# fboehm/DBSLMM

Measured on AMD Instinct MI355X. Metric: SNPs solved/sec (whole node) + max-|Δβ| vs CPU ref, 1M SNP × 10k indiv, higher is better.
Workload: dtype f64

## Files before the change

dbslmm_amd/csrc/pcg.hip:

```cpp
#include <hip/hip_runtime.h>
#include <stdint.h>

namespace pcg {
constexpr int kT = 128;
constexpr int kRunMax = 8;
constexpr int kMaxNC = 4;
constexpr int kWaves = 4;
constexpr int kVS = kT + 8;
constexpr int kNDot = 5;
constexpr int kQS = 8;
constexpr int kThreads = 256;
constexpr int kFTb = 8;
constexpr int kFRows = kFTb * kT;
constexpr int kFPer = kFRows / kThreads;
constexpr int wave_lds_doubles(int nc) { return 3 * nc * kVS + 4 * nc * 64; }
constexpr size_t lds_bytes(int nc) { return sizeof(double) * kWaves * wave_lds_doubles(nc); }
}

struct PcgBlk {
    int32_t blk, row0, m, ms;
    int32_t ld, Tb, Ns, sco;
    int64_t matoff, vo, po, dof;
    int64_t off16;
    int32_t nc;
    int32_t mshift;
    int32_t fused;
    int32_t pad_;
};

struct PcgArgs {
    const PcgBlk* blk;
    const uint16_t* G16;
    const double* M;
    const int32_t* flags;
    const double* S;
    const double* rsd;
    const double* z;
    const int32_t* slot_out;
    const int32_t* blk_id;
    const double* dshift;
    double *X, *R, *P, *Sv, *W;
    double* U;
    double* part;
    double* dot;
    double* qs;
    int32_t* cnv;
    int32_t* itb;
    int32_t* done;
    int32_t* active;
    int32_t* fin;
    double* beta_s;
    double* beta_l;
    int32_t* status;
    double* mir_s;
    double* mir_l;
    int32_t* mir_st;
    int32_t* mir_flag;
    int32_t run_no;
    int64_t vstride;
    int64_t ns, nl, nbk;
    double tau, rn, c0, tol, inv_sqrt_n;
    int32_t ncopy;
    int32_t run;
    int32_t seed;
};

namespace pcg {

__device__ __forceinline__ void wave_fence() {
    __builtin_amdgcn_fence(__ATOMIC_RELEASE, "wavefront");
    __builtin_amdgcn_wave_barrier();
    __builtin_amdgcn_fence(__ATOMIC_ACQUIRE, "wavefront");
}

template <int Ctrl>
__device__ __forceinline__ double dpp_mov(double v) {
    const uint64_t b = __builtin_bit_cast(uint64_t, v);
    const int lo = __builtin_amdgcn_mov_dpp(static_cast<int>(b & 0xffffffffu), Ctrl, 0xf, 0xf, false);
    const int hi = __builtin_amdgcn_mov_dpp(static_cast<int>(b >> 32), Ctrl, 0xf, 0xf, false);
    return __builtin_bit_cast(double, (static_cast<uint64_t>(static_cast<uint32_t>(hi)) << 32) | static_cast<uint32_t>(lo));
}
template <int X>
__device__ __forceinline__ uint32_t swap_xor(uint32_t x, bool up) {
    if constexpr (X == 16) {
        const auto r = __builtin_amdgcn_permlane16_swap(x, x, false, false);
        return up ? r[0] : r[1];
    } else {
        const auto r = __builtin_amdgcn_permlane32_swap(x, x, false, false);
        return up ? r[0] : r[1];
    }
}
template <int X>
__device__ __forceinline__ double lane_xor(double v) {
#ifndef PCG_NO_DPP
    if constexpr (X == 1) return dpp_mov<0xB1>(v);
    else if constexpr (X == 2) return dpp_mov<0x4E>(v);
    else if constexpr (X == 4) return dpp_mov<0x1B>(dpp_mov<0x141>(v));
    else if constexpr (X == 8) return dpp_mov<0x128>(v);
#ifndef PCG_NO_PERMLANE
    else if constexpr (X == 16 || X == 32) {
        const uint64_t b = __builtin_bit_cast(uint64_t, v);
        const bool up = (__lane_id() & X) != 0;
        const uint32_t lo = swap_xor<X>(static_cast<uint32_t>(b & 0xffffffffu), up);
        const uint32_t hi = swap_xor<X>(static_cast<uint32_t>(b >> 32), up);
        return __builtin_bit_cast(double, (static_cast<uint64_t>(hi) << 32) | lo);
    }
#endif
    else
#endif
        return __shfl_xor(v, X);
}

template <int X2, int X1, int X0>
__device__ __forceinline__ double rscatter8(const double (&v)[8], int lane) {
    const bool h2 = (lane & X2) != 0, h1 = (lane & X1) != 0, h0 = (lane & X0) != 0;
    double u[4], w[2];
#pragma unroll
    for (int q = 0; q < 4; ++q) {
        const double send = h2 ? v[q] : v[q + 4], keep = h2 ? v[q + 4] : v[q];
        u[q] = keep + lane_xor<X2>(send);
    }
#pragma unroll
    for (int q = 0; q < 2; ++q) {
        const double send = h1 ? u[q] : u[q + 2], keep = h1 ? u[q + 2] : u[q];
        w[q] = keep + lane_xor<X1>(send);
    }
    const double send = h0 ? w[0] : w[1], keep = h0 ? w[1] : w[0];
    return keep + lane_xor<X0>(send);
}

__device__ __forceinline__ double wave_sum(double v) {
    v += lane_xor<32>(v);
    v += lane_xor<16>(v);
    v += lane_xor<8>(v);
    v += lane_xor<4>(v);
    v += lane_xor<2>(v);
    v += lane_xor<1>(v);
    return v;
}



__device__ __forceinline__ double ordered_sum(const double* __restrict__ p, int64_t st, int s0, int s1, double acc) {
    for (int s = s0; s < s1; s += 8) {
        double t[8];
#pragma unroll
        for (int u = 0; u < 8; ++u) t[u] = s + u < s1 ? p[static_cast<int64_t>(s + u) * st] : 0.0;
#pragma unroll
        for (int u = 0; u < 8; ++u) acc += t[u];
    }
    return acc;
}

__device__ __forceinline__ bool on_u16(const PcgArgs& a, const PcgBlk& B) {
    return a.G16 != nullptr && (a.flags[B.blk] & 1) == 0;
}

__device__ __forceinline__ double jdiag(const PcgArgs& a, const PcgBlk& B, int i, double dc) {
    return B.mshift ? 1.0 : i < B.ms ? a.c0 + dc : a.c0;
}
__device__ __forceinline__ double col_shift(const PcgArgs& a, const PcgBlk& B, int k) {
    return a.dshift[B.mshift ? a.seed : k];
}

__device__ __forceinline__ void put_beta(const PcgArgs& a, const PcgBlk& B, int i, int k, double x, bool mono) {
    const int so = a.slot_out[B.row0 + i];
    const double bv = mono ? __builtin_nan("") : x * a.inv_sqrt_n;
    if (so >= 0) {
        a.beta_s[k * a.ns + so] = bv;
        if (a.mir_s) a.mir_s[k * a.ns + so] = bv;
    } else {
        a.beta_l[k * a.nl - 1 - so] = bv;
        if (a.mir_l) a.mir_l[k * a.nl - 1 - so] = bv;
    }
}
__device__ __forceinline__ void put_status(const PcgArgs& a, const PcgBlk& B, int k, bool mono) {
    const int st = mono ? DBSLMM_BLOCK_MONOMORPHIC
                        : a.cnv[B.sco + k] == 0 ? DBSLMM_BLOCK_NOT_CONVERGED : DBSLMM_BLOCK_OK;
    const int64_t o = k * a.nbk + a.blk_id[B.blk];
    a.status[o] = st;
    if (a.mir_st) a.mir_st[o] = st;
}

__device__ __forceinline__ double cvt_lo(uint32_t w) {
    double g;
    uint32_t t;
    asm volatile("v_and_b32 %1, 0xffff, %2\n\tv_cvt_f64_u32 %0, %1" : "=v"(g), "=&v"(t) : "v"(w));
    return g;
}
__device__ __forceinline__ double cvt_hi(uint32_t w) {
    double g;
    uint32_t t;
    asm volatile("v_lshrrev_b32 %1, 16, %2\n\tv_cvt_f64_u32 %0, %1" : "=v"(g), "=&v"(t) : "v"(w));
    return g;
}

typedef uint32_t pcg_u4 __attribute__((ext_vector_type(4)));

__device__ __forceinline__ __amdgpu_buffer_rsrc_t g16_rsrc(const uint16_t* base, uint32_t bytes) {
    const uint64_t gb = reinterpret_cast<uint64_t>(base);
    const uint32_t lo = static_cast<uint32_t>(__builtin_amdgcn_readfirstlane(static_cast<int>(gb & 0xffffffffu)));
    const uint32_t hi = static_cast<uint32_t>(__builtin_amdgcn_readfirstlane(static_cast<int>(gb >> 32)));
    const int nb = __builtin_amdgcn_readfirstlane(static_cast<int>(bytes));
    return __builtin_amdgcn_make_buffer_rsrc(reinterpret_cast<void*>((static_cast<uint64_t>(hi) << 32) | lo),
                                             static_cast<short>(0), nb, 0x00020000);
}
constexpr uint32_t kG16Oob = 0x80000000u;

__device__ __forceinline__ void quad_mul16(const pcg_u4 (&raw)[8], bool diagq, int lane, int nc,
                                           const double* vI, const double* vJ, double* rsum, double* csum) {
    const int rg = lane >> 3, cg = lane & 7;
#pragma unroll 1
    for (int k = 0; k < nc; ++k) {
        double vi[8], vj[8], racc[8], cacc[8];
#pragma unroll
        for (int q = 0; q < 8; ++q) {
            vi[q] = vI[k * kVS + 8 * rg + q];
            vj[q] = vJ[k * kVS + 8 * cg + q];
            racc[q] = cacc[q] = 0.0;
        }
        if (!diagq) {
#pragma unroll
            for (int r = 0; r < 8; ++r)
#pragma unroll
                for (int c = 0; c < 8; ++c) {
                    const uint32_t w = raw[r][c >> 1];
                    const double g = (c & 1) ? cvt_hi(w) : cvt_lo(w);
                    racc[r] = __builtin_fma(g, vj[c], racc[r]);
                    cacc[c] = __builtin_fma(g, vi[r], cacc[c]);
                }
        } else {
#pragma unroll
            for (int r = 0; r < 8; ++r)
#pragma unroll
                for (int c = 0; c < 8; ++c) {
                    const uint32_t w = raw[r][c >> 1];
                    const double g = (c & 1) ? cvt_hi(w) : cvt_lo(w);
                    const int dd = 8 * (cg - rg) + c - r;
                    racc[r] = __builtin_fma(dd <= 0 ? g : 0.0, vj[c], racc[r]);
                    cacc[c] = __builtin_fma(dd < 0 ? g : 0.0, vi[r], cacc[c]);
                }
        }
        rsum[k * 64 + lane] += rscatter8<4, 2, 1>(racc, lane);
        csum[k * 64 + lane] += rscatter8<32, 16, 8>(cacc, lane);
    }
}

__device__ __forceinline__ void quad_mul64(const double* __restrict__ base, int64_t ld, int rows_ok, int cols_ok,
                                           bool diagq, int lane, int nc, const double* vI, const double* vJ,
                                           double* rsum, double* csum) {
    const int rg = lane >> 3, cg = lane & 7;
#pragma unroll 1
    for (int k = 0; k < nc; ++k) {
        double vi[8], vj[8], racc[8], cacc[8];
#pragma unroll
        for (int q = 0; q < 8; ++q) {
            vi[q] = vI[k * kVS + 8 * rg + q];
            vj[q] = vJ[k * kVS + 8 * cg + q];
            racc[q] = cacc[q] = 0.0;
        }
#pragma unroll 1
        for (int r = 0; r < 8; ++r)
#pragma unroll
            for (int c = 0; c < 8; ++c) {
                const double g = (r < rows_ok && c < cols_ok) ? base[r * ld + c] : 0.0;
                const int dd = 8 * (cg - rg) + c - r;
                const double gr = !diagq || dd <= 0 ? g : 0.0, gc = !diagq || dd < 0 ? g : 0.0;
#pragma unroll
                for (int q = 0; q < 8; ++q)
                    if (q == r) racc[q] = __builtin_fma(gr, vj[c], racc[q]);
                cacc[c] = __builtin_fma(gc, vi[r], cacc[c]);
            }
        rsum[k * 64 + lane] += rscatter8<4, 2, 1>(racc, lane);
        csum[k * 64 + lane] += rscatter8<32, 16, 8>(cacc, lane);
    }
}

__device__ __forceinline__ void stage_v(const PcgArgs& a, const PcgBlk& B, int T, int nc, int lane, double* v) {
    for (int k = 0; k < nc; ++k) {
        const double* src = a.U + k * a.vstride + B.vo + static_cast<int64_t>(T) * kT;
        const double x0 = src[lane], x1 = src[lane + 64];
        v[k * kVS + lane] = x0;
        v[k * kVS + lane + 64] = x1;
    }
}

__device__ __forceinline__ bool quad_active(const PcgBlk& B, int I, int J, int q) {
    const int qi = q >> 1, qj = q & 1;
    return !(J == I && qj > qi) && I * kT + 64 * qi < B.m && J * kT + 64 * qj < B.m;
}
__device__ __forceinline__ bool next_quad(const PcgBlk& B, int I, int J1, int& J, int& q) {
    for (;;) {
        if (++q == 4) {
            q = 0;
            if (++J > J1) return false;
        }
        if (quad_active(B, I, J, q)) return true;
    }
}

template <bool U16>
__device__ void symv_item(const PcgArgs& a, int4 item, int lane, double* vI, double* vJb, double* rsum,
                          double* csum) {
    const PcgBlk B = a.blk[item.x];
    if (a.done[item.x] || on_u16(a, B) != U16) return;
    const int I = item.y, J0 = item.z, J1 = item.w, nc = B.nc;
    const int64_t ld16 = static_cast<int64_t>(B.Tb) * kT;
    const int rg = lane >> 3, cg = lane & 7;
    auto vj_of = [&](int J) -> double* { return J == I ? vI : vJb + ((J - J0) & 1) * nc * kVS; };
    const __amdgpu_buffer_rsrc_t g16 =
        g16_rsrc(a.G16 + B.off16 + static_cast<int64_t>(I) * kT * ld16, U16 ? static_cast<uint32_t>(kT * ld16 * 2) : 0u);
    auto load = [&](int J, int q, pcg_u4 (&raw)[8], bool none) {
        if constexpr (U16) {
            const int i0 = 64 * (q >> 1) + 8 * rg, j0 = J * kT + 64 * (q & 1) + 8 * cg;
            const bool skip = none || j0 >= B.m || (J == I && (q == 0 || q == 3) && cg > rg);
            const uint32_t o = static_cast<uint32_t>((static_cast<int64_t>(i0) * ld16 + j0) * 2);
#pragma unroll
            for (int r = 0; r < 8; ++r)
                raw[r] = __builtin_amdgcn_raw_buffer_load_b128(
                    g16, (skip || I * kT + i0 + r >= B.m) ? kG16Oob : o + static_cast<uint32_t>(r * ld16 * 2), 0, 0);
        }
    };
    auto mult = [&](int J, int q, const pcg_u4 (&raw)[8]) {
        const int qi = q >> 1, qj = q & 1;
        const bool dq = J == I && qi == qj;
        const double* vj = vj_of(J);
        double* rs = rsum + qi * nc * 64;
        double* cs = csum + qj * nc * 64;
        if constexpr (U16) {
            quad_mul16(raw, dq, lane, nc, vI + 64 * qi, vj + 64 * qj, rs, cs);
        } else {
            const int ib = I * kT + 64 * qi + 8 * rg, jb = J * kT + 64 * qj + 8 * cg;
            quad_mul64(a.M + B.matoff + static_cast<int64_t>(ib) * B.ld + jb, B.ld, B.m - ib, B.m - jb, dq,
                       lane, nc, vI + 64 * qi, vj + 64 * qj, rs, cs);
        }
    };
    auto flush = [&](int J) {
        double* dst = a.part + B.po + (static_cast<int64_t>(J) * B.Ns + I) * nc * kT;
        for (int qj = 0; qj < 2; ++qj)
            for (int k = 0; k < nc; ++k) {
                dst[k * kT + 64 * qj + 8 * cg + rg] = csum[(qj * nc + k) * 64 + lane];
                csum[(qj * nc + k) * 64 + lane] = 0.0;
            }
    };
    pcg_u4 ra[8], rb[8];
    int J = J0, q = 0;
    load(J, q, ra, false);
    stage_v(a, B, I, nc, lane, vI);
    if (J != I) stage_v(a, B, J, nc, lane, vj_of(J));
    for (int t = 0; t < 2 * nc; ++t) rsum[t * 64 + lane] = csum[t * 64 + lane] = 0.0;
    wave_fence();
    auto step = [&](pcg_u4 (&cur)[8], pcg_u4 (&nxt)[8]) -> bool {
        int Jn = J, qn = q;
        const bool more = next_quad(B, I, J1, Jn, qn);
        load(more ? Jn : J, more ? qn : q, nxt, !more);
        if (more && Jn != J && Jn != I) stage_v(a, B, Jn, nc, lane, vj_of(Jn));
        mult(J, q, cur);
        if (!more || Jn != J) flush(J);
        wave_fence();
        J = Jn;
        q = qn;
        return more;
    };
    while (step(ra, rb) && step(rb, ra)) {
    }
    double* dst = a.part + B.po + (static_cast<int64_t>(I) * B.Ns + B.Tb + J0 / a.run) * nc * kT;
    for (int qi = 0; qi < 2; ++qi)
        for (int k = 0; k < nc; ++k) dst[k * kT + 64 * qi + 8 * rg + cg] = rsum[(qi * nc + k) * 64 + lane];
}

}

extern "C" __global__ __launch_bounds__(pcg::kThreads) void dbslmm_pcg_init(PcgArgs a, const int2* __restrict__ rows) {
    using namespace pcg;
    __shared__ double red[kThreads / 64][kMaxNC];
    __shared__ int mono_s;
    const int2 it = rows[blockIdx.x];
    const int bi = it.x, I = it.y, tid = threadIdx.x;
    const PcgBlk B = a.blk[bi];
    const bool u16 = on_u16(a, B);
    const int n = a.ncopy, nc = B.nc;
    if (I == 0) {
        if (tid == 0) mono_s = 0;
        __syncthreads();
        bool mono = false;
        for (int i = tid; i < B.m; i += kThreads) mono |= !(a.rsd[B.row0 + i] < INFINITY);
        if (mono) atomicOr(&mono_s, 1);
        __syncthreads();
        if (tid < n) {
            a.cnv[B.sco + tid] = 0;
            double* q = a.qs + static_cast<int64_t>(B.sco + tid) * kQS;
            q[4] = q[5] = 1.0;
        }
        if (tid == 0) {
            a.itb[bi] = 0;
            a.fin[bi] = 0;
            const bool fz = B.fused && u16;
            a.done[bi] = mono_s ? 2 : fz ? 3 : 0;
            if (!mono_s && !fz) atomicAdd(a.active, 1);
        }
    }
    const int r = tid & (kT - 1), h = tid >> 7, i = I * kT + r;
    const bool in = i < B.m;
    double sv[kMaxNC];
#pragma unroll
    for (int k = 0; k < kMaxNC; ++k) sv[k] = 0.0;
    for (int c = h; c < n; c += 2) {
        const int64_t o = c * a.vstride + B.vo + i;
        const double rhs = in ? a.z[B.row0 + i] : 0.0;
        a.X[o] = 0.0;
        a.P[o] = 0.0;
        if (c < nc) {
            a.Sv[o] = 0.0;
            a.W[o] = 0.0;
            a.R[o] = rhs;
            double uv = 0.0;
            if (in) {
                uv = rhs / jdiag(a, B, i, col_shift(a, B, c));
                if (u16) uv *= a.rsd[B.row0 + i];
            }
            a.U[o] = uv;
        }
    }
#pragma unroll
    for (int k = 0; k < kMaxNC; ++k)
        if (k < nc && (k & 1) == h && in && u16) {
            const double rhs = a.z[B.row0 + i];
            sv[k] = a.S[B.row0 + i] * a.rsd[B.row0 + i] * (rhs / jdiag(a, B, i, col_shift(a, B, k)));
        }
#pragma unroll
    for (int k = 0; k < kMaxNC; ++k) sv[k] = wave_sum(sv[k]);
    if ((tid & 63) == 0)
#pragma unroll
        for (int k = 0; k < kMaxNC; ++k) red[tid >> 6][k] = sv[k];
    __syncthreads();
    if (tid < nc) {
        const int hk = tid & 1;
        a.dot[B.dof + (static_cast<int64_t>(I) * kNDot + 4) * n + tid] = red[2 * hk][tid] + red[2 * hk + 1][tid];
    }
}

template <bool U16>
__device__ __forceinline__ void symv_body(const PcgArgs& a, const int4* __restrict__ items, int32_t n_items) {
    using namespace pcg;
    extern __shared__ double vlds[];
    const int wave = threadIdx.x >> 6, lane = threadIdx.x & 63;
    const int e = blockIdx.x * kWaves + wave;
    if (e >= n_items) return;
    const int nc = a.ncopy;
    double* w = vlds + wave * wave_lds_doubles(nc);
    symv_item<U16>(a, items[e], lane, w, w + nc * kVS, w + 3 * nc * kVS, w + 3 * nc * kVS + 2 * nc * 64);
}
#ifndef PCG_SYMV_WAVES
#define PCG_SYMV_WAVES 2
#endif
extern "C" __global__ __launch_bounds__(pcg::kThreads) __attribute__((amdgpu_waves_per_eu(PCG_SYMV_WAVES, 8)))
void dbslmm_pcg_symv16(PcgArgs a, const int4* __restrict__ items, int32_t n_items) {
    symv_body<true>(a, items, n_items);
}
extern "C" __global__ __launch_bounds__(pcg::kThreads)
void dbslmm_pcg_symv64(PcgArgs a, const int4* __restrict__ items, int32_t n_items) {
    symv_body<false>(a, items, n_items);
}

extern "C" __global__ __launch_bounds__(pcg::kThreads) void dbslmm_pcg_rows(PcgArgs a, const int2* __restrict__ rows) {
    using namespace pcg;
    __shared__ double red[kThreads / 64][kMaxNC][4];
    __shared__ double sig[kMaxNC];
    const int2 it = rows[blockIdx.x];
    const int bi = it.x, I = it.y, tid = threadIdx.x;
    if (a.done[bi]) return;
    const PcgBlk B = a.blk[bi];
    const bool u16 = on_u16(a, B);
    const int n = a.ncopy, nc = B.nc;
    if (tid < nc)
        sig[tid] = ordered_sum(a.dot + B.dof + 4 * n + tid, kNDot * n, 0, B.Tb, 0.0);
    __syncthreads();
    const int r = tid & (kT - 1), h = tid >> 7, i = I * kT + r;
    const bool in = i < B.m;
    const double Si = in ? a.S[B.row0 + i] : 0.0, ri = in ? a.rsd[B.row0 + i] : 0.0;
    const int nrun = (I + a.run) / a.run;
    double dv[kMaxNC][4];
#pragma unroll
    for (int k = 0; k < kMaxNC; ++k)
#pragma unroll
        for (int f = 0; f < 4; ++f) dv[k][f] = 0.0;
#pragma unroll
    for (int k = 0; k < kMaxNC; ++k) {
        if (k >= n || (k & 1) != h) continue;
        const int64_t o = k * a.vstride + B.vo + i;
        if (k < nc) {
            const double* pp = a.part + B.po + static_cast<int64_t>(I) * B.Ns * nc * kT + k * kT + r;
            double y = ordered_sum(pp, nc * kT, I, B.Tb, 0.0);
            y = ordered_sum(pp, nc * kT, B.Tb, B.Tb + nrun, y);
            const double dc = col_shift(a, B, k);
            const double rv = a.R[o];
            const double u = in ? rv / jdiag(a, B, i, dc) : 0.0;
            const double sh = i < B.ms ? dc : 0.0;
            double w = 0.0;
            if (in) {
                if (u16) w = a.tau * a.rn * ri * __builtin_fma(-Si, sig[k] * a.rn, y) + (1.0 - a.tau + sh) * u;
                else w = y + sh * u;
            }
            a.W[o] = w;
            dv[k][0] = rv * u;
            dv[k][1] = w * u;
            dv[k][2] = rv * rv;
        }
        const double xv = a.X[o];
        dv[k][3] = xv * xv;
    }
#pragma unroll
    for (int k = 0; k < kMaxNC; ++k)
#pragma unroll
        for (int f = 0; f < 4; ++f) dv[k][f] = wave_sum(dv[k][f]);
    if ((tid & 63) == 0)
#pragma unroll
        for (int k = 0; k < kMaxNC; ++k)
#pragma unroll
            for (int f = 0; f < 4; ++f) red[tid >> 6][k][f] = dv[k][f];
    __syncthreads();
    if (tid < 4 * n) {
        const int k = tid >> 2, f = tid & 3, hk = k & 1;
        if (f == 3 || k < nc)
            a.dot[B.dof + (static_cast<int64_t>(I) * kNDot + f) * n + k] = red[2 * hk][k][f] + red[2 * hk + 1][k][f];
    }
    if (I == 0 && tid == 0) a.itb[bi] += 1;
}

extern "C" __global__ __launch_bounds__(pcg::kThreads) void dbslmm_pcg_update(PcgArgs a, const int2* __restrict__ rows) {
    using namespace pcg;
    __shared__ double tot[kMaxNC][4];
    __shared__ double coef[kMaxNC][3];
    __shared__ double seedc[2];
    __shared__ int run_s[kMaxNC];
    __shared__ double red[kThreads / 64][kMaxNC];
    const int2 it = rows[blockIdx.x];
    const int bi = it.x, I = it.y, tid = threadIdx.x;
    if (a.done[bi]) return;
    const PcgBlk B = a.blk[bi];
    const bool u16 = on_u16(a, B);
    const int n = a.ncopy, nc = B.nc;
    const int itn = a.itb[bi] - 1;
    const int par = itn & 1;
    if (tid < 4 * n) {
        const int k = tid >> 2, f = tid & 3;
        tot[k][f] = (f == 3 || k < nc) ? ordered_sum(a.dot + B.dof + f * n + k, kNDot * n, 0, B.Tb, 0.0) : 0.0;
    }
    __syncthreads();
    if (B.mshift) {
        if (tid == 0) {
            const double gam = tot[0][0], del = tot[0][1];
            const double* q = a.qs + static_cast<int64_t>(B.sco) * kQS;
            double al, be = 0.0;
            if (itn == 0) {
                al = gam / del;
            } else {
                be = gam / q[2 * par];
                al = gam / (del - be * gam / q[2 * par + 1]);
            }
            seedc[0] = al;
            seedc[1] = be;
        }
        __syncthreads();
        if (tid < n) {
            const int c = tid;
            double* q = a.qs + static_cast<int64_t>(B.sco + c) * kQS;
            const double al = seedc[0], be = seedc[1];
            const double zk = q[4 + 2 * par], zk1 = q[4 + 2 * par + 1];
            const double rr = tot[0][2] * zk * zk, xx = tot[c][3];
            const double t = a.tol * (a.dshift[c] + 1.0 - a.tau);
            const bool conv = a.cnv[B.sco + c] != 0 || rr == 0.0 || rr <= t * t * xx;
            const double e = a.dshift[c] - a.dshift[a.seed];
            const double cp = itn == 0 ? 0.0 : al * be / a.qs[static_cast<int64_t>(B.sco) * kQS + 2 * par + 1];
            const double zn = zk * zk1 / ((1.0 + cp + al * e) * zk1 - cp * zk);
            coef[c][0] = al * zn / zk;
            coef[c][1] = zk1 != 0.0 ? (zk / zk1) * (zk / zk1) * be : 0.0;
            coef[c][2] = zk;
            run_s[c] = conv ? 0 : 1;
            if (I == 0) {
                if (conv && a.cnv[B.sco + c] == 0) a.cnv[B.sco + c] = itn + 1;
                q[4 + 2 * (par ^ 1)] = zn;
                q[4 + 2 * (par ^ 1) + 1] = zk;
            }
        }
        __syncthreads();
        if (I == 0 && tid == 0) {
            double* q = a.qs + static_cast<int64_t>(B.sco) * kQS;
            q[2 * (par ^ 1)] = tot[0][0];
            q[2 * (par ^ 1) + 1] = seedc[0];
        }
    } else {
        if (tid < n) {
            const int k = tid;
            const double gam = tot[k][0], del = tot[k][1], rr = tot[k][2], xx = tot[k][3];
            const double lam = B.ms == B.m ? a.dshift[k] + 1.0 - a.tau : 1.0 - a.tau;
            const double t = a.tol * lam;
            const bool conv = a.cnv[B.sco + k] != 0 || rr == 0.0 || rr <= t * t * xx;
            double al = 0.0, be = 0.0;
            if (!conv) {
                double* q = a.qs + static_cast<int64_t>(B.sco + k) * kQS;
                if (itn == 0) {
                    al = gam / del;
                } else {
                    be = gam / q[2 * par];
                    al = gam / (del - be * gam / q[2 * par + 1]);
                }
                if (I == 0) {
                    q[2 * (par ^ 1)] = gam;
                    q[2 * (par ^ 1) + 1] = al;
                }
            } else if (I == 0 && a.cnv[B.sco + k] == 0) {
                a.cnv[B.sco + k] = itn + 1;
            }
            coef[k][0] = al;
            coef[k][1] = be;
            coef[k][2] = 1.0;
            run_s[k] = conv ? 0 : 1;
        }
        __syncthreads();
    }
    int running = 0;
    for (int k = 0; k < n; ++k) running += run_s[k];
    if (running == 0) {
        const int r = tid & (kT - 1), h = tid >> 7, i = I * kT + r;
        if (i < B.m)
            for (int k = h; k < n; k += 2) put_beta(a, B, i, k, a.X[k * a.vstride + B.vo + i], false);
        if (I == 0 && tid < n) put_status(a, B, tid, false);
        __syncthreads();
        if (tid == 0 &&
            __hip_atomic_fetch_add(a.fin + bi, 1, __ATOMIC_ACQ_REL, __HIP_MEMORY_SCOPE_AGENT) == B.Tb - 1) {
            a.done[bi] = 1;
            atomicSub(a.active, 1);
            if (a.mir_flag)
                for (int c = 0; c < n; ++c)
                    __hip_atomic_store(a.mir_flag + static_cast<int64_t>(bi) * n + c, a.run_no, __ATOMIC_RELEASE,
                                       __HIP_MEMORY_SCOPE_SYSTEM);
        }
        return;
    }
    const int r = tid & (kT - 1), h = tid >> 7, i = I * kT + r;
    const bool in = i < B.m;
    double sv[kMaxNC];
#pragma unroll
    for (int k = 0; k < kMaxNC; ++k) sv[k] = 0.0;
    if (B.mshift) {
        if (in) {
            const int64_t o0 = B.vo + i;
            const double rv = a.R[o0];
#pragma unroll
            for (int c = 0; c < kMaxNC; ++c) {
                if (c >= n || (c & 1) != h || !run_s[c]) continue;
                const int64_t o = c * a.vstride + o0;
                const double p = __builtin_fma(coef[c][1], a.P[o], coef[c][2] * rv);
                a.P[o] = p;
                a.X[o] = __builtin_fma(coef[c][0], p, a.X[o]);
            }
            if (h == 0) {
                const double al = seedc[0], be = seedc[1];
                const double sn = __builtin_fma(be, a.Sv[o0], a.W[o0]);
                const double rn = __builtin_fma(-al, sn, rv);
                a.Sv[o0] = sn;
                a.R[o0] = rn;
                a.U[o0] = u16 ? rn * a.rsd[B.row0 + i] : rn;
                if (u16) sv[0] = a.S[B.row0 + i] * a.rsd[B.row0 + i] * rn;
            }
        }
    } else {
#pragma unroll
        for (int k = 0; k < kMaxNC; ++k) {
            if (k >= n || (k & 1) != h || !run_s[k] || !in) continue;
            const int64_t o = k * a.vstride + B.vo + i;
            const double al = coef[k][0], be = coef[k][1];
            const double dg = jdiag(a, B, i, a.dshift[k]);
            const double u = a.R[o] / dg;
            const double p = __builtin_fma(be, a.P[o], u);
            const double s = __builtin_fma(be, a.Sv[o], a.W[o]);
            const double x = __builtin_fma(al, p, a.X[o]);
            const double rn = __builtin_fma(-al, s, a.R[o]);
            a.P[o] = p;
            a.Sv[o] = s;
            a.X[o] = x;
            a.R[o] = rn;
            a.U[o] = u16 ? (rn / dg) * a.rsd[B.row0 + i] : rn / dg;
            if (u16) sv[k] = a.S[B.row0 + i] * a.rsd[B.row0 + i] * (rn / dg);
        }
    }
#pragma unroll
    for (int k = 0; k < kMaxNC; ++k) sv[k] = wave_sum(sv[k]);
    if ((tid & 63) == 0)
#pragma unroll
        for (int k = 0; k < kMaxNC; ++k) red[tid >> 6][k] = sv[k];
    __syncthreads();
    if (tid < nc && (B.mshift || run_s[tid])) {
        const int hk = tid & 1;
        a.dot[B.dof + (static_cast<int64_t>(I) * kNDot + 4) * n + tid] = red[2 * hk][tid] + red[2 * hk + 1][tid];
    }
}

#ifndef PCG_BLOCK_DEPTH
#define PCG_BLOCK_DEPTH 3
#endif
namespace pcg {
template <int N>
__device__ __forceinline__ void block_sum(double (&v)[N], double* red, int tid) {
#pragma unroll
    for (int k = 0; k < N; ++k) v[k] = wave_sum(v[k]);
    __syncthreads();
    if ((tid & 63) == 0)
#pragma unroll
        for (int k = 0; k < N; ++k) red[(tid >> 6) * N + k] = v[k];
    __syncthreads();
#pragma unroll
    for (int k = 0; k < N; ++k) v[k] = ((red[k] + red[N + k]) + red[2 * N + k]) + red[3 * N + k];
}
constexpr size_t block_lds_bytes(int n) {
    return sizeof(double) * ((5 + 2 * n) * kFRows + 4 * (3 + kMaxNC) + 12 + 3 * kMaxNC + 4);
}
}

__device__ __forceinline__ void pcg_block_solve(const PcgArgs& a, int bi, int cc, int32_t maxit) {
    using namespace pcg;
    extern __shared__ double blds[];
    double* yw = blds;
    double* Ul = blds + 4 * kFRows;
    const int n = a.ncopy;
    double* Xl = Ul + kFRows;
    double* Pl = Xl + n * kFRows;
    double* red = Pl + n * kFRows;
    if (a.done[bi] != 3) return;
    const PcgBlk B = a.blk[bi];
    const int tid = threadIdx.x, lane = tid & 63, wave = tid >> 6;
    const int m = B.m, Tb = B.Tb;
    const bool msh = cc < 0;
    const int nx = msh ? n : 1;
    const double dc = msh ? col_shift(a, B, 0) : a.dshift[cc];
    double r[kFPer], sv[kFPer], wv[kFPer], Sr[kFPer], Rr[kFPer], sg[1] = {0.0};
#pragma unroll
    for (int q = 0; q < kFPer; ++q) {
        const int i = tid + kThreads * q;
        const bool in = i < m;
        r[q] = in ? a.z[B.row0 + i] : 0.0;
        Sr[q] = in ? a.S[B.row0 + i] : 0.0;
        Rr[q] = in ? a.rsd[B.row0 + i] : 0.0;
        sv[q] = wv[q] = 0.0;
        double u = 0.0;
        if (in) {
            u = (r[q] / jdiag(a, B, i, dc)) * Rr[q];
            sg[0] += Sr[q] * u;
        }
        Ul[i] = u;
        for (int w = 0; w < 4; ++w) yw[w * kFRows + i] = 0.0;
        for (int c = 0; c < nx; ++c) Xl[c * kFRows + i] = Pl[c * kFRows + i] = 0.0;
    }
    block_sum(sg, red, tid);
    double sig = sg[0];
    const int Q = (m + 63) / 64;
    const int nq = Q * (Q + 1) / 2;
    const int64_t ld16 = static_cast<int64_t>(Tb) * kT;
    const int rg = lane >> 3, cg = lane & 7;
    auto quad_of = [&](int t, int& qi, int& qj) {
        qi = static_cast<int>((sqrtf(8.0f * t + 1.0f) - 1.0f) * 0.5f);
        while (qi * (qi + 1) / 2 > t) --qi;
        while ((qi + 1) * (qi + 2) / 2 <= t) ++qi;
        qj = t - qi * (qi + 1) / 2;
    };
    const __amdgpu_buffer_rsrc_t g16 = g16_rsrc(a.G16 + B.off16, static_cast<uint32_t>(ld16 * ld16 * 2));
    auto load = [&](int t, pcg_u4 (&raw)[8]) {
        int qi, qj;
        quad_of(t, qi, qj);
        const int r0 = 64 * qi + 8 * rg, c0 = 64 * qj + 8 * cg;
        const bool skip = t >= nq || c0 >= m || (qi == qj && cg > rg);
        const uint32_t o = static_cast<uint32_t>((r0 * static_cast<int>(ld16) + c0) * 2);
#pragma unroll
        for (int rr = 0; rr < 8; ++rr)
            raw[rr] = __builtin_amdgcn_raw_buffer_load_b128(
                g16, (skip || r0 + rr >= m) ? kG16Oob : o + static_cast<uint32_t>(rr * ld16 * 2), 0, 0);
    };
    auto mult = [&](int t, const pcg_u4 (&raw)[8]) {
        int qi, qj;
        quad_of(t, qi, qj);
        const bool dq = qi == qj;
        double vi[8], vj[8], racc[8], cacc[8];
#pragma unroll
        for (int q = 0; q < 8; ++q) {
            vi[q] = Ul[64 * qi + 8 * rg + q];
            vj[q] = Ul[64 * qj + 8 * cg + q];
            racc[q] = cacc[q] = 0.0;
        }
        if (!dq) {
#pragma unroll
            for (int rr = 0; rr < 8; ++rr)
#pragma unroll
                for (int c = 0; c < 8; ++c) {
                    const uint32_t w = raw[rr][c >> 1];
                    const double g = (c & 1) ? cvt_hi(w) : cvt_lo(w);
                    racc[rr] = __builtin_fma(g, vj[c], racc[rr]);
                    cacc[c] = __builtin_fma(g, vi[rr], cacc[c]);
                }
        } else {
#pragma unroll
            for (int rr = 0; rr < 8; ++rr)
#pragma unroll
                for (int c = 0; c < 8; ++c) {
                    const uint32_t w = raw[rr][c >> 1];
                    const double g = (c & 1) ? cvt_hi(w) : cvt_lo(w);
                    const int dd = 8 * (cg - rg) + c - rr;
                    racc[rr] = __builtin_fma(dd <= 0 ? g : 0.0, vj[c], racc[rr]);
                    cacc[c] = __builtin_fma(dd < 0 ? g : 0.0, vi[rr], cacc[c]);
                }
        }
        double* y = yw + wave * kFRows;
        const int ri = 64 * qi + 8 * rg + cg, ci = 64 * qj + 8 * cg + rg;
        y[ri] += rscatter8<4, 2, 1>(racc, lane);
        wave_fence();
        y[ci] += rscatter8<32, 16, 8>(cacc, lane);
    };
    double* st = red + 4 * (3 + kMaxNC);
    int* flag = reinterpret_cast<int*>(st + 12 + 3 * kMaxNC);
    if (tid == 0) {
        for (int c = 0; c < kMaxNC; ++c) {
            st[4 + c] = st[8 + c] = 1.0;
            flag[c] = c >= n;
        }
    }
    int it = 0;
    for (; it < maxit; ++it) {
        __syncthreads();
        {
#if PCG_BLOCK_DEPTH == 3
            pcg_u4 ra[8], rb[8], rc[8];
            int t = wave;
            load(t, ra);
            load(t + 4, rb);
            while (t < nq) {
                load(t + 8, rc);
                mult(t, ra);
                t += 4;
                if (t >= nq) break;
                load(t + 8, ra);
                mult(t, rb);
                t += 4;
                if (t >= nq) break;
                load(t + 8, rb);
                mult(t, rc);
                t += 4;
            }
#else
            pcg_u4 ra[8], rb[8];
            int t = wave;
            load(t, ra);
            while (t < nq) {
                load(t + 4, rb);
                mult(t, ra);
                t += 4;
                if (t >= nq) break;
                load(t + 4, ra);
                mult(t, rb);
                t += 4;
            }
#endif
        }
        __syncthreads();
        double d[3 + kMaxNC];
#pragma unroll
        for (int k = 0; k < 3 + kMaxNC; ++k) d[k] = 0.0;
#pragma unroll
        for (int q = 0; q < kFPer; ++q) {
            const int i = tid + kThreads * q;
            double y = 0.0;
            if (i < Tb * kT) {
                y = ((yw[i] + yw[kFRows + i]) + yw[2 * kFRows + i]) + yw[3 * kFRows + i];
#pragma unroll
                for (int w = 0; w < 4; ++w) yw[w * kFRows + i] = 0.0;
            }
            if (i < m) {
                const double Si = Sr[q], ri = Rr[q];
                const double u = r[q] / jdiag(a, B, i, dc);
                const double sh = i < B.ms ? dc : 0.0;
                const double w = a.tau * a.rn * ri * __builtin_fma(-Si, sig * a.rn, y) + (1.0 - a.tau + sh) * u;
                wv[q] = w;
                d[0] += r[q] * u;
                d[1] += w * u;
                d[2] += r[q] * r[q];
                for (int c = 0; c < nx; ++c) {
                    const double xv = Xl[c * kFRows + i];
                    d[3 + c] += xv * xv;
                }
            }
        }
        block_sum(d, red, tid);
        if (tid == 0) {
            const double gam = d[0], del = d[1], rr = d[2];
            double al, be = 0.0;
            if (it == 0) {
                al = gam / del;
            } else {
                be = gam / st[0];
                al = gam / (del - be * gam / st[1]);
            }
            int running = 0;
            if (msh) {
                const double cp = it == 0 ? 0.0 : al * be / st[1];
                for (int c = 0; c < n; ++c) {
                    const double zk = st[4 + c], zk1 = st[8 + c];
                    const double t = a.tol * (a.dshift[c] + 1.0 - a.tau);
                    const double rrc = rr * zk * zk;
                    if (!flag[c] && (rrc == 0.0 || rrc <= t * t * d[3 + c])) {
                        flag[c] = 1;
                        a.cnv[B.sco + c] = it + 1;
                    }
                    const double e = a.dshift[c] - a.dshift[a.seed];
                    const double zn = zk * zk1 / ((1.0 + cp + al * e) * zk1 - cp * zk);
                    st[12 + 3 * c] = al * zn / zk;
                    st[12 + 3 * c + 1] = zk1 != 0.0 ? (zk / zk1) * (zk / zk1) * be : 0.0;
                    st[12 + 3 * c + 2] = zk;
                    st[8 + c] = zk;
                    st[4 + c] = zn;
                    running += flag[c] ? 0 : 1;
                }
            } else {
                const double lam = B.ms == B.m ? dc + 1.0 - a.tau : 1.0 - a.tau;
                const double t = a.tol * lam;
                if (rr == 0.0 || rr <= t * t * d[3]) {
                    flag[0] = 1;
                    a.cnv[B.sco + cc] = it + 1;
                }
                running = flag[0] ? 0 : 1;
            }
            st[0] = gam;
            st[1] = al;
            st[2] = al;
            st[3] = be;
            flag[kMaxNC] = running;
        }
        __syncthreads();
        if (flag[kMaxNC] == 0) break;
        const double al = st[2], be = st[3];
        double sg2[1] = {0.0};
#pragma unroll
        for (int q = 0; q < kFPer; ++q) {
            const int i = tid + kThreads * q;
            if (i >= m) continue;
            const double rsd_i = Rr[q];
            double rn;
            if (msh) {
                for (int c = 0; c < n; ++c) {
                    if (flag[c]) continue;
                    const int o = c * kFRows + i;
                    const double pv = __builtin_fma(st[12 + 3 * c + 1], Pl[o], st[12 + 3 * c + 2] * r[q]);
                    Pl[o] = pv;
                    Xl[o] = __builtin_fma(st[12 + 3 * c], pv, Xl[o]);
                }
                const double sn = __builtin_fma(be, sv[q], wv[q]);
                rn = __builtin_fma(-al, sn, r[q]);
                sv[q] = sn;
                r[q] = rn;
                Ul[i] = rn * rsd_i;
            } else {
                const double dg = jdiag(a, B, i, dc);
                const double u = r[q] / dg;
                const double pv = __builtin_fma(be, Pl[i], u);
                const double sn = __builtin_fma(be, sv[q], wv[q]);
                Pl[i] = pv;
                Xl[i] = __builtin_fma(al, pv, Xl[i]);
                rn = __builtin_fma(-al, sn, r[q]);
                sv[q] = sn;
                r[q] = rn;
                Ul[i] = (rn / dg) * rsd_i;
            }
            sg2[0] += Sr[q] * Ul[i];
        }
        block_sum(sg2, red, tid);
        sig = sg2[0];
    }
#pragma unroll
    for (int q = 0; q < kFPer; ++q) {
        const int i = tid + kThreads * q;
        if (i < m)
            for (int c = 0; c < nx; ++c) put_beta(a, B, i, msh ? c : cc, Xl[c * kFRows + i], false);
    }
    if (tid == 0) {
        atomicMax(a.itb + bi, it + (it < maxit ? 1 : 0));
        for (int c = 0; c < nx; ++c) put_status(a, B, msh ? c : cc, false);
    }
    if (a.mir_flag) {
        __syncthreads();
        if (tid == 0)
            for (int c = 0; c < nx; ++c)
                __hip_atomic_store(a.mir_flag + static_cast<int64_t>(bi) * n + (msh ? c : cc), a.run_no,
                                   __ATOMIC_RELEASE, __HIP_MEMORY_SCOPE_SYSTEM);
    }
}

extern "C" __global__ __launch_bounds__(pcg::kThreads)
#if PCG_BLOCK_DEPTH == 3
__attribute__((amdgpu_waves_per_eu(1, 8), amdgpu_num_vgpr(312)))
#else
__attribute__((amdgpu_waves_per_eu(2, 8)))
#endif
void dbslmm_pcg_block(PcgArgs a, const int2* __restrict__ list, int32_t n_list, int32_t* __restrict__ next,
                      int32_t maxit) {
    __shared__ int e_s;
    for (;;) {
        __syncthreads();
        if (threadIdx.x == 0) e_s = atomicAdd(next, 1);
        __syncthreads();
        const int e = e_s;
        if (e >= n_list) break;
        pcg_block_solve(a, list[e].x, list[e].y, maxit);
    }
}

extern "C" __global__ __launch_bounds__(pcg::kThreads) void dbslmm_pcg_final(PcgArgs a, const int2* __restrict__ rows) {
    using namespace pcg;
    const int2 it = rows[blockIdx.x];
    const int bi = it.x, I = it.y, tid = threadIdx.x;
    const int done = a.done[bi];
    if (done == 3 || done == 1) return;
    const PcgBlk B = a.blk[bi];
    const bool mono = done == 2;
    const int r = tid & (kT - 1), h = tid >> 7, i = I * kT + r;
    if (i < B.m)
        for (int k = h; k < a.ncopy; k += 2) put_beta(a, B, i, k, a.X[k * a.vstride + B.vo + i], mono);
    if (I == 0 && tid < a.ncopy) put_status(a, B, tid, mono);
}
```

Measured before the change: 157.1 million.

## Prefetch first G16 tiles across PCG iterations and track quad positions incrementally

Replaces the per-tile triangular index computation (sqrtf plus correction loops) with an incrementally advanced (t, qi, qj) position. The first two tile loads are issued before the setup phase and are re-issued at the tail of each iteration, so the next iteration starts with its data already in flight. The loop is restructured around a per-wave tile count with a scalarized wave index, and the depth-2 compile option is removed. This hides load latency at the start of each PCG iteration and cuts address arithmetic, in exchange for holding three register tile buffers live across the whole iteration body.

Result: faster. 160.9 million (median of 6 runs) (+2.4%).

```diff
diff --git a/dbslmm_amd/csrc/pcg.hip b/dbslmm_amd/csrc/pcg.hip
--- a/dbslmm_amd/csrc/pcg.hip
+++ b/dbslmm_amd/csrc/pcg.hip
@@ -698,9 +698,6 @@
     }
 }
 
-#ifndef PCG_BLOCK_DEPTH
-#define PCG_BLOCK_DEPTH 3
-#endif
 namespace pcg {
 template <int N>
 __device__ __forceinline__ void block_sum(double (&v)[N], double* red, int tid) {
@@ -730,11 +727,45 @@
     double* red = Pl + n * kFRows;
     if (a.done[bi] != 3) return;
     const PcgBlk B = a.blk[bi];
-    const int tid = threadIdx.x, lane = tid & 63, wave = tid >> 6;
+    const int tid = threadIdx.x, lane = tid & 63;
+    const int wave = __builtin_amdgcn_readfirstlane(tid >> 6);
     const int m = B.m, Tb = B.Tb;
     const bool msh = cc < 0;
     const int nx = msh ? n : 1;
     const double dc = msh ? col_shift(a, B, 0) : a.dshift[cc];
+    const int Q = (m + 63) / 64;
+    const int nq = Q * (Q + 1) / 2;
+    const int nw = (nq + 3 - wave) >> 2;
+    const int64_t ld16 = static_cast<int64_t>(Tb) * kT;
+    const int rg = lane >> 3, cg = lane & 7;
+    struct QPos {
+        int t, qi, qj;
+    };
+    auto adv = [](QPos& p, int k) {
+        p.t += k;
+        p.qj += k;
+        while (p.qj > p.qi) {
+            p.qj -= p.qi + 1;
+            ++p.qi;
+        }
+    };
+    QPos first{0, 0, 0};
+    adv(first, wave);
+    QPos second = first;
+    adv(second, 4);
+    const __amdgpu_buffer_rsrc_t g16 = g16_rsrc(a.G16 + B.off16, static_cast<uint32_t>(ld16 * ld16 * 2));
+    auto load = [&](const QPos& p, pcg_u4 (&raw)[8]) {
+        const int r0 = 64 * p.qi + 8 * rg, c0 = 64 * p.qj + 8 * cg;
+        const bool skip = p.t >= nq || c0 >= m || (p.qi == p.qj && cg > rg);
+        const uint32_t o = static_cast<uint32_t>((r0 * static_cast<int>(ld16) + c0) * 2);
+#pragma unroll
+        for (int rr = 0; rr < 8; ++rr)
+            raw[rr] = __builtin_amdgcn_raw_buffer_load_b128(
+                g16, (skip || r0 + rr >= m) ? kG16Oob : o + static_cast<uint32_t>(rr * ld16 * 2), 0, 0);
+    };
+    pcg_u4 ra[8], rb[8], rc[8];
+    load(first, ra);
+    load(second, rb);
     double r[kFPer], sv[kFPer], wv[kFPer], Sr[kFPer], Rr[kFPer], sg[1] = {0.0};
 #pragma unroll
     for (int q = 0; q < kFPer; ++q) {
@@ -755,31 +786,8 @@
     }
     block_sum(sg, red, tid);
     double sig = sg[0];
-    const int Q = (m + 63) / 64;
-    const int nq = Q * (Q + 1) / 2;
-    const int64_t ld16 = static_cast<int64_t>(Tb) * kT;
-    const int rg = lane >> 3, cg = lane & 7;
-    auto quad_of = [&](int t, int& qi, int& qj) {
-        qi = static_cast<int>((sqrtf(8.0f * t + 1.0f) - 1.0f) * 0.5f);
-        while (qi * (qi + 1) / 2 > t) --qi;
-        while ((qi + 1) * (qi + 2) / 2 <= t) ++qi;
-        qj = t - qi * (qi + 1) / 2;
-    };
-    const __amdgpu_buffer_rsrc_t g16 = g16_rsrc(a.G16 + B.off16, static_cast<uint32_t>(ld16 * ld16 * 2));
-    auto load = [&](int t, pcg_u4 (&raw)[8]) {
-        int qi, qj;
-        quad_of(t, qi, qj);
-        const int r0 = 64 * qi + 8 * rg, c0 = 64 * qj + 8 * cg;
-        const bool skip = t >= nq || c0 >= m || (qi == qj && cg > rg);
-        const uint32_t o = static_cast<uint32_t>((r0 * static_cast<int>(ld16) + c0) * 2);
-#pragma unroll
-        for (int rr = 0; rr < 8; ++rr)
-            raw[rr] = __builtin_amdgcn_raw_buffer_load_b128(
-                g16, (skip || r0 + rr >= m) ? kG16Oob : o + static_cast<uint32_t>(rr * ld16 * 2), 0, 0);
-    };
-    auto mult = [&](int t, const pcg_u4 (&raw)[8]) {
-        int qi, qj;
-        quad_of(t, qi, qj);
+    auto mult = [&](const QPos& p, const pcg_u4 (&raw)[8]) {
+        const int qi = p.qi, qj = p.qj;
         const bool dq = qi == qj;
         double vi[8], vj[8], racc[8], cacc[8];
 #pragma unroll
@@ -828,38 +836,36 @@
     for (; it < maxit; ++it) {
         __syncthreads();
         {
-#if PCG_BLOCK_DEPTH == 3
-            pcg_u4 ra[8], rb[8], rc[8];
-            int t = wave;
-            load(t, ra);
-            load(t + 4, rb);
-            while (t < nq) {
-                load(t + 8, rc);
-                mult(t, ra);
-                t += 4;
-                if (t >= nq) break;
-                load(t + 8, ra);
-                mult(t, rb);
-                t += 4;
-                if (t >= nq) break;
-                load(t + 8, rb);
-                mult(t, rc);
-                t += 4;
-            }
-#else
-            pcg_u4 ra[8], rb[8];
-            int t = wave;
-            load(t, ra);
-            while (t < nq) {
-                load(t + 4, rb);
-                mult(t, ra);
-                t += 4;
-                if (t >= nq) break;
-                load(t + 4, ra);
-                mult(t, rb);
-                t += 4;
-            }
-#endif
+            QPos pm = first, pl = second;
+            adv(pl, 4);
+            int s = 0;
+            for (; s + 3 < nw; s += 3) {
+                load(pl, rc);
+                adv(pl, 4);
+                mult(pm, ra);
+                adv(pm, 4);
+                load(pl, ra);
+                adv(pl, 4);
+                mult(pm, rb);
+                adv(pm, 4);
+                load(pl, rb);
+                adv(pl, 4);
+                mult(pm, rc);
+                adv(pm, 4);
+            }
+            if (nw > 0) {
+                const int rem = nw - s;
+                load(pl, rc);
+                mult(pm, ra);
+                adv(pm, 4);
+                load(first, ra);
+                if (rem >= 2) {
+                    mult(pm, rb);
+                    adv(pm, 4);
+                }
+                load(second, rb);
+                if (rem >= 3) mult(pm, rc);
+            }
         }
         __syncthreads();
         double d[3 + kMaxNC];
@@ -994,11 +1000,7 @@
 }
 
 extern "C" __global__ __launch_bounds__(pcg::kThreads)
-#if PCG_BLOCK_DEPTH == 3
 __attribute__((amdgpu_waves_per_eu(1, 8), amdgpu_num_vgpr(312)))
-#else
-__attribute__((amdgpu_waves_per_eu(2, 8)))
-#endif
 void dbslmm_pcg_block(PcgArgs a, const int2* __restrict__ list, int32_t n_list, int32_t* __restrict__ next,
                       int32_t maxit) {
     __shared__ int e_s;
```
